# blyssprivacy/sdk

Hardware: NVIDIA H100
Metric: PIR server queries/sec (Spiral process_query) (higher is better)
Workload: dtype u64

## Files before the change

### sdk_b200/build.py

```python
import os
import subprocess
import sys

HERE = os.path.dirname(os.path.abspath(__file__))
CSRC = os.path.join(HERE, "csrc")
SO = os.path.join(HERE, "libb200pir.so")
SOURCES = ["api.cu", "poly_kernels.cu", "mul_kernels.cu", "imma_kernels.cu", "wire_kernels.cu", "tc5_kernels.cu", "dpir_gemm.cu"]
HEADERS = ["common.cuh", "kernels.h", "ntt_core.cuh", "tc5_layout.cuh", "tc5_ptx.cuh", "ntt_core4096.cuh", "ntt_tables.hpp", os.path.join("..", "..", "include", "b200pir.h")]
NVCC_FLAGS = ["-gencode", "arch=compute_90a,code=sm_90a", "-lineinfo", "-O3", "-std=c++17", "--extended-lambda",
              "-Xcompiler", "-fPIC", "-ccbin", "/usr/bin/g++" if os.path.exists("/usr/bin/g++") else "g++"]


def _stale():
    if not os.path.exists(SO):
        return True
    t = os.path.getmtime(SO)
    return any(os.path.getmtime(os.path.join(CSRC, f)) > t for f in SOURCES + HEADERS)


def build(force=False, verbose=False):
    if not force and not _stale():
        return SO
    nvcc = os.environ.get("NVCC", "/usr/local/cuda/bin/nvcc")
    objs = []
    procs = []
    for src in SOURCES:
        obj = os.path.join(CSRC, src.replace(".cu", ".o"))
        cmd = [nvcc] + NVCC_FLAGS + (["-Xptxas", "-v"] if verbose else []) + ["-c", os.path.join(CSRC, src), "-o", obj]
        procs.append((src, subprocess.Popen(cmd, stdout=subprocess.PIPE, stderr=subprocess.STDOUT, text=True)))
        objs.append(obj)
    for src, p in procs:
        out, _ = p.communicate()
        if verbose or p.returncode:
            sys.stderr.write(out)
        if p.returncode:
            raise RuntimeError("nvcc failed on " + src)
    subprocess.check_call([nvcc, "-shared", "-gencode", "arch=compute_90a,code=sm_90a", "-o", SO] + objs + ["-ccbin", NVCC_FLAGS[-1]])
    return SO


if __name__ == "__main__":
# ... 2 lines not shown
```

### sdk_b200/csrc/poly_kernels.cu

```cuda
#include "kernels.h"
#include "ntt_core4096.cuh"

namespace b200pir {

namespace {

constexpr int CTA = 512;
constexpr int HI_TW = NTT_N - 64;

__constant__ Twiddle c_tw_lo[2][3][64];

struct TwConst {
  int n, dir;
  __device__ __forceinline__ Twiddle operator()(int i) const { return c_tw_lo[n][dir][i]; }
  __device__ __forceinline__ void load2(int i, Twiddle (&t)[2]) const { t[0] = (*this)(i); t[1] = (*this)(i + 1); }
  __device__ __forceinline__ void load4(int i, Twiddle (&t)[4]) const {
    t[0] = (*this)(i); t[1] = (*this)(i + 1); t[2] = (*this)(i + 2); t[3] = (*this)(i + 3);
  }
};
struct TwShared {
  const Twiddle* p;
  __device__ __forceinline__ Twiddle operator()(int i) const { return p[i - 64]; }
  __device__ __forceinline__ void load2(int i, Twiddle (&t)[2]) const {
    uint4 v = *reinterpret_cast<const uint4*>(p + (i - 64));
    t[0] = Twiddle{v.x, v.y}; t[1] = Twiddle{v.z, v.w};
  }
  __device__ __forceinline__ void load4(int i, Twiddle (&t)[4]) const {
    uint4 v = *reinterpret_cast<const uint4*>(p + (i - 64)), w = *(reinterpret_cast<const uint4*>(p + (i - 64)) + 1);
    t[0] = Twiddle{v.x, v.y}; t[1] = Twiddle{v.z, v.w}; t[2] = Twiddle{w.x, w.y}; t[3] = Twiddle{w.z, w.w};
  }
};
struct TwGlobal {
  const Twiddle* p;
  __device__ __forceinline__ Twiddle operator()(int i) const {
// ... 140 lines not shown
#pragma unroll
        for (int e = 0; e < 8; e++) acc[r][e] += (uint64_t)x1[e] * cv[e];
      }
    }
  }
#pragma unroll 1
  for (; k < ndig; k++) {
    uint32_t x[8];
#pragma unroll
    for (int a = 0; a < 8; a++) x[a] = gadget_digit_fast<BYTE>(v(a), k, bits, mask);
    if (SM) ntt_forward_group_lz<NTT_OUT_LAZY16>(g.tid, x, g.smem, TwConst{g.n, 0}, TwShared{g.fwd_hi_sm}, g.q, CtaSync());
    else ntt_forward_group_lz<NTT_OUT_LAZY16>(g.tid, x, g.smem, TwConst{g.n, 0}, TwGlobal{g.fwd}, g.q, CtaSync());
    if (cnt + 1 > 16) { acc_reduce<ROWS>(acc, g); cnt = 1; }
    cnt += 1;
    const uint32_t* c = c0 + (size_t)k * col_step;
#pragma unroll
    for (int r = 0; r < ROWS; r++) {
      uint32_t cv[8];
      ld8_ro(cv, c + (size_t)r * row_step);
#pragma unroll
      for (int e = 0; e < 8; e++) acc[r][e] += (uint64_t)x[e] * cv[e];
    }
  }
}

template <int ROWS, bool SM, typename Coef>
__device__ __forceinline__ void digits_mac(uint64_t (&acc)[ROWS][8], int& cnt, Coef v, int ndig,
                                           int bits, const uint32_t* c0, size_t col_step, size_t row_step,
                                           const Grp& g) {
  if (bits == 8) digits_mac_impl<ROWS, SM, true>(acc, cnt, v, ndig, bits, c0, col_step, row_step, g);
  else digits_mac_impl<ROWS, SM, false>(acc, cnt, v, ndig, bits, c0, col_step, row_step, g);
}

template <typename Sink>
__device__ __forceinline__ void crt_lift(const uint32_t (&x)[8], uint32_t* res, const Grp& g, const DevParams& P,
                                         Sink sink) {
  __syncthreads();
#pragma unroll
  for (int a = 0; a < 8; a++) res[g.n * POLY + a * 256 + g.tid] = x[a];
  __syncthreads();
#pragma unroll
  for (int a4 = 0; a4 < 4; a4++) {
    int z = (g.n * 4 + a4) * 256 + g.tid;
    sink(z, crt_compose(res[z], res[POLY + z], P));
  }
}

__global__ void __launch_bounds__(256) k_ntt32(DevParams P, uint32_t* polys, int inverse) {
  __shared__ __align__(16) uint32_t ntt_smem[NTT_SMEM_WORDS];
  Grp g = make_grp_single(P, ntt_smem, blockIdx.y);
  uint32_t* p = polys + ((size_t)blockIdx.x * 2 + g.n) * POLY;
  uint32_t x[8];
  if (!inverse) {
#pragma unroll
    for (int a = 0; a < 8; a++) x[a] = p[a * 256 + g.tid];
    grp_ntt_fwd<false>(g, x);
    st8(p + g.tid * 8, x);
  } else {
    ld8(x, p + g.tid * 8);
    grp_ntt_inv(g, x);
#pragma unroll
    for (int a = 0; a < 8; a++) p[a * 256 + g.tid] = x[a];
  }
}
__global__ void __launch_bounds__(NTT4K_THREADS)
k_ntt32_4k(uint32_t q0, uint32_t q1, const Twiddle* __restrict__ tw , uint32_t* polys, int inverse) {
// ... 106 lines not shown
    const uint64_t* ct = base + (size_t)(src == 0 ? i : half + i) * 2 * POLY;
    const uint32_t* C = (src == 0 ? c_neg : c_pos) + qoff;
#pragma unroll 1
    for (int rho = 0; rho < 2; rho++) {
      uint64_t v[8];
#pragma unroll
      for (int a = 0; a < 8; a++) v[a] = ct[rho * POLY + a * 256 + g.tid];
      const uint32_t* c0 = C + ((size_t)rho * 2 + g.n) * POLY + g.tid * 8;
      digits_mac<2, false>(acc, cnt, RegCoef{v}, t_gsw, bits, c0, col_step, row_step, g);
    }
  }
  uint64_t* dst = base + (size_t)i * 2 * POLY;
#pragma unroll 1
  for (int r = 0; r < 2; r++) {
    uint32_t x[8];
#pragma unroll
    for (int e = 0; e < 8; e++) x[e] = barrett64(acc[r][e], g.cr1, g.q);
    grp_ntt_inv(g, x);
    uint64_t* d = dst + r * POLY;
    crt_lift(x, res, g, P, [&](int z, uint64_t val) { d[z] = val; });
  }
}

__device__ __forceinline__ uint32_t digit_diff(uint64_t vh, uint64_t vi, int k, int bits, uint64_t mask, uint32_t q) {
  return gadget_digit(vh, k, bits, mask) - gadget_digit(vi, k, bits, mask) + q;
}
__device__ __forceinline__ uint32_t byte_pair_diff(uint64_t vh, uint64_t vi, int k) {
  const uint32_t sel = 0x7070u | ((uint32_t)(k + 1) << 8) | (uint32_t)k;
  return __byte_perm((uint32_t)vh, (uint32_t)(vh >> 32), sel) + 0x01000100u -
         __byte_perm((uint32_t)vi, (uint32_t)(vi >> 32), sel);
}
constexpr int kFoldPlanes = 4;

template <bool BYTE>
__global__ void __launch_bounds__(256, 2)
k_fold_res_lz(DevParams P, const uint32_t* __restrict__ in, uint32_t* __restrict__ out, size_t batch_stride, int half,
              const uint32_t* __restrict__ c_pos, size_t c_batch_stride, int slices_per_query, int t_gsw, int bits,
              const uint32_t* __restrict__ zero_flags ) {
  if (zero_flags) {
    const int bz = blockIdx.x / half, iz = blockIdx.x % half;
    const uint32_t fa = zero_flags[(size_t)bz * 2 * half + iz], fb = zero_flags[(size_t)bz * 2 * half + half + iz];
    if (fa | fb) {
      const uint32_t* src = in + (size_t)bz * batch_stride + (size_t)((fa ? half : 0) + iz) * 4 * POLY;
      uint32_t* dst = out + (size_t)bz * batch_stride + (size_t)iz * 4 * POLY;
#pragma unroll
      for (int rho = 0; rho < 2; rho++) {
        uint32_t x[8];
        ld8_ro(x, src + ((size_t)rho * 2 + blockIdx.y) * POLY + threadIdx.x * 8);
        st8(dst + ((size_t)rho * 2 + blockIdx.y) * POLY + threadIdx.x * 8, x);
      }
      return;
    }
  }
  extern __shared__ __align__(16) uint8_t dyn_smem[];
  uint32_t* sm0 = reinterpret_cast<uint32_t*>(dyn_smem);
  uint32_t* sm1 = sm0 + NTT_SMEM_WORDS;
  Twiddle* tw = reinterpret_cast<Twiddle*>(sm1 + NTT_SMEM_WORDS);
  Grp g = make_grp_single(P, sm0, blockIdx.y);
  stage_fwd_twiddles(g, tw);
  const TwConst lo{g.n, 0};
  const TwShared hi{tw};
  const int b = blockIdx.x / half, i = blockIdx.x % half;
  const uint32_t* ci = in + (size_t)b * batch_stride + (size_t)i * 4 * POLY;
  const uint32_t* ch = in + (size_t)b * batch_stride + (size_t)(half + i) * 4 * POLY;
  const uint32_t* C = c_pos + (size_t)(b / slices_per_query) * c_batch_stride;
  const int cols = 2 * t_gsw;
  const size_t row_step = (size_t)cols * 2 * POLY;
  const uint64_t mask = (1ull << bits) - 1;
  const uint32_t q = g.q;
  uint32_t* planes = reinterpret_cast<uint32_t*>(tw + HI_TW) + g.tid;

  uint64_t acc[2][8];
#pragma unroll
  for (int r = 0; r < 2; r++)
#pragma unroll
    for (int e = 0; e < 8; e++) acc[r][e] = 0;
  int cnt = 0;
#pragma unroll 1
  for (int rho = 0; rho < 2; rho++) {
    uint64_t vi[8], vh[8];
#pragma unroll
    for (int a = 0; a < 8; a++) {
      const int z = a * 256 + g.tid;
      vi[a] = crt_compose(__ldg(ci + (rho * 2 + 0) * POLY + z), __ldg(ci + (rho * 2 + 1) * POLY + z), P);
      vh[a] = crt_compose(__ldg(ch + (rho * 2 + 0) * POLY + z), __ldg(ch + (rho * 2 + 1) * POLY + z), P);
      if (BYTE) {
#pragma unroll
        for (int p = 0; p < kFoldPlanes; p++)
          if (2 * p < t_gsw) planes[p * POLY + a * 256] = byte_pair_diff(vh[a], vi[a], 2 * p);
      }
    }
    const uint32_t* c0 = C + ((size_t)rho * 2 + g.n) * POLY + g.tid * 8;
    int k = 0;
#pragma unroll 1
    for (; k + 1 < t_gsw; k += 2) {
      uint32_t x0[8], x1[8];
#pragma unroll
      for (int a = 0; a < 8; a++) {
        if (BYTE) {
          const uint32_t w = planes[(k >> 1) * POLY + a * 256];
          x0[a] = (w & 0xffffu) + (q - 256u);
          x1[a] = (w >> 16) + (q - 256u);
        } else {
          x0[a] = digit_diff(vh[a], vi[a], k, bits, mask, q);
          x1[a] = digit_diff(vh[a], vi[a], k + 1, bits, mask, q);
        }
      }
      ntt_forward_group2_lz<NTT_OUT_LAZY16>(g.tid, x0, x1, sm0, sm1, lo, hi, q, CtaSync());
      if (cnt + 2 > 16) { acc_reduce<2>(acc, g); cnt = 1; }
      cnt += 2;
#pragma unroll
      for (int r = 0; r < 2; r++) {
        uint32_t cv[8];
        ld8_ro(cv, c0 + (size_t)r * row_step + (size_t)k * 4 * POLY);
#pragma unroll
        for (int e = 0; e < 8; e++) acc[r][e] += (uint64_t)x0[e] * cv[e];
      }
#pragma unroll
      for (int r = 0; r < 2; r++) {
        uint32_t cv[8];
        ld8_ro(cv, c0 + (size_t)r * row_step + (size_t)(k + 1) * 4 * POLY);
#pragma unroll
        for (int e = 0; e < 8; e++) acc[r][e] += (uint64_t)x1[e] * cv[e];
      }
    }
    if (k < t_gsw) {
      uint32_t x0[8];
#pragma unroll
      for (int a = 0; a < 8; a++)
        x0[a] = BYTE ? (planes[(k >> 1) * POLY + a * 256] & 0xffffu) + (q - 256u) : digit_diff(vh[a], vi[a], k, bits, mask, q);
      ntt_forward_group_lz<NTT_OUT_LAZY16>(g.tid, x0, sm0, lo, hi, q, CtaSync());
      if (cnt + 1 > 16) { acc_reduce<2>(acc, g); cnt = 1; }
      cnt += 1;
#pragma unroll
      for (int r = 0; r < 2; r++) {
        uint32_t cv[8];
        ld8_ro(cv, c0 + (size_t)r * row_step + (size_t)k * 4 * POLY);
#pragma unroll
        for (int e = 0; e < 8; e++) acc[r][e] += (uint64_t)x0[e] * cv[e];
      }
    }
  }
  uint32_t y0[8], y1[8];
#pragma unroll
  for (int e = 0; e < 8; e++) {
    y0[e] = barrett64(acc[0][e], g.cr1, q);
    y1[e] = barrett64(acc[1][e], g.cr1, q);
  }
  ntt_inverse_group2_nh(g.tid, y0, y1, sm0, sm1, TwConst{g.n, 2}, TwGlobal{g.inv_lz}, q, CtaSync());
  uint32_t* co = out + (size_t)b * batch_stride + (size_t)i * 4 * POLY;
#pragma unroll
  for (int a = 0; a < 8; a++) {
    const int z = a * 256 + g.tid;
    co[(0 * 2 + g.n) * POLY + z] = addmod(y0[a], __ldg(ci + (0 * 2 + g.n) * POLY + z), q);
    co[(1 * 2 + g.n) * POLY + z] = addmod(y1[a], __ldg(ci + (1 * 2 + g.n) * POLY + z), q);
  }
}

__global__ void __launch_bounds__(256)
k_ct_zero_flags(const uint32_t* __restrict__ cts, size_t batch_stride, int per_batch, uint32_t* __restrict__ flags) {
  const int b = blockIdx.x / per_batch, idx = blockIdx.x % per_batch;
  const uint4* p = reinterpret_cast<const uint4*>(cts + (size_t)b * batch_stride + (size_t)idx * 4 * POLY);
  uint32_t acc = 0;
#pragma unroll
  for (int k = 0; k < 8; k++) {
    const uint4 v = __ldg(p + k * 256 + threadIdx.x);
    acc |= v.x | v.y | v.z | v.w;
  }
  const int any = __syncthreads_or(acc != 0);
  if (threadIdx.x == 0) flags[blockIdx.x] = any ? 0u : 1u;
}

__global__ void k_folding_neg(DevParams P, uint32_t* out, const uint32_t* vf, size_t total, int t_gsw, int bits) {
  size_t idx = (size_t)blockIdx.x * blockDim.x + threadIdx.x;
  if (idx >= total) return;
  int n = (int)((idx / POLY) & 1);
  size_t poly = idx / (2 * POLY);
  int cols = 2 * t_gsw;
  int c = (int)(poly % cols);
  int r = (int)((poly / cols) & 1);
  uint32_t q = P.q[n];
  uint32_t v = vf[idx];
  uint32_t neg = v == 0 ? 0u : q - v;
  uint32_t gval = 0;
  if ((c & 1) == r) {
    int j = c >> 1;
    if (bits * j < 64) gval = barrett64(1ull << (bits * j), P.cr1[n], q);
  }
  out[idx] = addmod(neg, gval, q);
// ... 186 lines not shown
            const unsigned ee = 2u * (__brev(sidx) >> (32 - NTT_LOG_N)) + 1u;
            const unsigned e2 = (ee * (unsigned)R.t_auto) & (2u * POLY - 1u);
            const unsigned src = __brev((e2 - 1u) >> 1) >> (32 - NTT_LOG_N);
            yy = barrett64((uint64_t)yy * __ldg(ng + src), g.cr1, g.q);
          }
          s = addmod(s, yy, g.q);
        }
        o[e] = s;
      }
      st8(dst + ((size_t)rho * 2 + g.n) * POLY + g.tid * 8, o);
    }
    __syncthreads();
  }
}

__global__ void __launch_bounds__(256)
k_expand_intt(DevParams P, const uint32_t* __restrict__ v, size_t v_stride, uint32_t* __restrict__ xr, size_t xr_stride,
              ExpandRound R) {
  __shared__ __align__(16) uint32_t ntt_smem[NTT_SMEM_WORDS];
  const int i = blockIdx.x;
  if ((R.stop_round > 0 && R.r > R.stop_round && (i & 1)) ||
      (R.stop_round > 0 && R.r == R.stop_round && (i & 1) && (i / 2) >= R.max_bits_to_gen_right))
    return;
  Grp g = make_grp_single(P, ntt_smem, blockIdx.y);
  const uint32_t* src = v + (size_t)blockIdx.z * v_stride + ((size_t)i * 4 + g.n) * POLY;
  uint32_t x[8];
  ld8_ro(x, src + g.tid * 8);
  grp_ntt_inv(g, x);
  uint32_t* dst = xr + (size_t)blockIdx.z * xr_stride + ((size_t)i * 2 + g.n) * POLY;
#pragma unroll
  for (int a = 0; a < 8; a++) dst[a * 256 + g.tid] = x[a];
}

__global__ void __launch_bounds__(256, 2)
k_expand_round_res(DevParams P, uint32_t* v, size_t v_stride, const uint32_t* __restrict__ xr, size_t xr_stride,
                   ExpandRound R, const uint32_t* __restrict__ neg1) {
  v += (size_t)blockIdx.z * v_stride;
  xr += (size_t)blockIdx.z * xr_stride;
  extern __shared__ __align__(16) uint8_t dyn_smem[];
  uint32_t* sm0 = reinterpret_cast<uint32_t*>(dyn_smem);
  uint32_t* sm1 = sm0 + NTT_SMEM_WORDS;
  uint64_t* autom = reinterpret_cast<uint64_t*>(sm1 + NTT_SMEM_WORDS);
  Twiddle* tw = reinterpret_cast<Twiddle*>(autom + POLY);
  Grp g = make_grp_single(P, sm0, blockIdx.y);
  g.smem2 = sm1;
  const int i = blockIdx.x;
  const uint32_t* ng = neg1 + (size_t)g.n * POLY;
  uint32_t* vi = v + (size_t)i * 4 * POLY;
  uint32_t* vo = v + (size_t)(i + R.num_in) * 4 * POLY;
  if ((R.stop_round > 0 && R.r > R.stop_round && (i & 1)) ||
      (R.stop_round > 0 && R.r == R.stop_round && (i & 1) && (i / 2) >= R.max_bits_to_gen_right)) {
    if (R.fill_skipped) {
      uint32_t nn[8];
      ld8_ro(nn, ng + g.tid * 8);
#pragma unroll
      for (int rho = 0; rho < 2; rho++) {
        uint32_t x[8];
        ld8(x, vi + ((size_t)rho * 2 + g.n) * POLY + g.tid * 8);
#pragma unroll
        for (int e = 0; e < 8; e++) x[e] = barrett64((uint64_t)x[e] * nn[e], g.cr1, g.q);
        st8(vo + ((size_t)rho * 2 + g.n) * POLY + g.tid * 8, x);
      }
    }
    return;
  }
  const bool left = (R.r != 0) && ((i & 1) == 0);
  const uint32_t* W = left ? R.tab_left[blockIdx.z] + R.off_left : R.tab_right[blockIdx.z] + R.off_right;
  const int t_exp = left ? R.t_left : R.t_right;
  const int bits = left ? R.bits_left : R.bits_right;
  stage_fwd_twiddles(g, tw);
  const uint32_t* x0r = xr + (size_t)i * 2 * POLY;
  const uint32_t* x1r = x0r + POLY;
  const uint32_t* row1 = vi + ((size_t)2 + g.n) * POLY;
  const uint64_t Q = P.modulus;
  const uint32_t q0 = P.q[0], q1 = P.q[1];
#pragma unroll 1
  for (int half = 1; half >= 0; half--) {
    const int shift = half ? R.num_in : 0;
#pragma unroll
    for (int a = 0; a < 8; a++) {
      const int k = a * 256 + g.tid;
      const int zs = (k + shift) & (POLY - 1);
      uint32_t a0 = __ldg(x0r + zs), a1 = __ldg(x1r + zs);
      if (k + shift >= POLY) {
        a0 = a0 ? q0 - a0 : 0u;
        a1 = a1 ? q1 - a1 : 0u;
      }
      const uint64_t val = crt_compose(a0, a1, P);
      const unsigned prod = (unsigned)k * (unsigned)R.t_auto;
      const unsigned num = prod >> NTT_LOG_N, rem = prod & (POLY - 1);
      autom[rem] = (num & 1u) ? Q - val : val;
    }
    __syncthreads();
    uint64_t acc[2][8];
#pragma unroll
    for (int r = 0; r < 2; r++)
#pragma unroll
      for (int e = 0; e < 8; e++) acc[r][e] = 0;
    int cnt = 0;
    digits_mac<2, true>(acc, cnt, SmemCoef{autom + g.tid}, t_exp, bits, W + (size_t)g.n * POLY + g.tid * 8, (size_t)2 * POLY,
                        (size_t)t_exp * 2 * POLY, g);
    uint32_t yy[8];
#pragma unroll
    for (int e = 0; e < 8; e++) {
      const unsigned sidx = (unsigned)(g.tid * 8 + e);
      const unsigned ee = 2u * (__brev(sidx) >> (32 - NTT_LOG_N)) + 1u;
      const unsigned e2 = (ee * (unsigned)R.t_auto) & (2u * POLY - 1u);
      const unsigned src = __brev((e2 - 1u) >> 1) >> (32 - NTT_LOG_N);
      uint32_t t = row1[src];
      if (half) t = barrett64((uint64_t)t * __ldg(ng + src), g.cr1, g.q);
      yy[e] = t;
    }
    __syncthreads();
    uint32_t* dst = half ? vo : vi;
    uint32_t nn[8];
    if (half) ld8_ro(nn, ng + g.tid * 8);
#pragma unroll
    for (int rho = 0; rho < 2; rho++) {
      uint32_t o[8];
      ld8(o, vi + ((size_t)rho * 2 + g.n) * POLY + g.tid * 8);
#pragma unroll
      for (int e = 0; e < 8; e++) {
        uint32_t base = o[e];
        if (half) base = barrett64((uint64_t)base * nn[e], g.cr1, g.q);
        uint32_t s = addmod(base, barrett64(acc[rho][e], g.cr1, g.q), g.q);
        o[e] = rho ? addmod(s, yy[e], g.q) : s;
      }
      st8(dst + ((size_t)rho * 2 + g.n) * POLY + g.tid * 8, o);
    }
  }
}

__global__ void k_reorient(MulGeom G, uint4* q_dev, size_t q_stride, const uint32_t* v, size_t v_stride, int idx_factor) {
  q_dev += (size_t)blockIdx.y * q_stride;
  v += (size_t)blockIdx.y * v_stride;
  size_t idx = (size_t)blockIdx.x * blockDim.x + threadIdx.x;
  if (idx >= (size_t)G.dim0 * POLY) return;
  int z = (int)(idx % POLY), j = (int)(idx / POLY);
  const uint32_t* ct = v + (size_t)idx_factor * j * 4 * POLY;
  uint4 o = make_uint4(ct[z], ct[POLY + z], ct[2 * POLY + z], ct[3 * POLY + z]);
  q_dev[((size_t)(j >> 1) * 2 + (j & 1)) * POLY + z] = o;
}

__global__ void __launch_bounds__(CTA, 1)
k_regev_to_gsw(DevParams P, uint32_t* v_gsw, size_t gsw_stride, const uint32_t* v, size_t v_stride, int idx_factor,
               int idx_offset, const uint32_t* const* tab_conv, int t_gsw, int t_conv, int bits_conv) {
  const uint32_t* v_conv = tab_conv[blockIdx.y];
  v_gsw += (size_t)blockIdx.y * gsw_stride;
  v += (size_t)blockIdx.y * v_stride;
  extern __shared__ __align__(16) uint8_t dyn_smem[];
  uint32_t* ntt_smem = reinterpret_cast<uint32_t*>(dyn_smem);
  uint32_t* res = ntt_smem + 4 * NTT_SMEM_WORDS;
  uint64_t* raw = reinterpret_cast<uint64_t*>(res + 2 * POLY);
  Twiddle* tw = reinterpret_cast<Twiddle*>(raw + 2 * POLY);
  Grp g = make_grp(P, ntt_smem);
  g.smem2 = ntt_smem + (2 + g.n) * NTT_SMEM_WORDS;
  stage_fwd_twiddles(g, tw + g.n * HI_TW);
  const int i = blockIdx.x / t_gsw, j = blockIdx.x % t_gsw;
  const int idx_inp = idx_factor * (i * t_gsw + j) + idx_offset;
  const uint32_t* inp = v + (size_t)idx_inp * 4 * POLY;
  const int cols = 2 * t_gsw;
  uint32_t* out = v_gsw + (size_t)i * 2 * cols * 2 * POLY;
#pragma unroll 1
// ... 157 lines not shown
  const uint64_t inst_bits = first_cnt * q2_bits + rest_cnt * q1_bits;
  uint64_t lo_bit = (uint64_t)w * 64, hi_bit = lo_bit + 64;
  uint64_t word = 0;
  uint64_t bit = lo_bit;
  while (bit < hi_bit) {
    uint64_t inst = bit / inst_bits;
    if (inst >= (uint64_t)instances) break;
    uint64_t off = bit - inst * inst_bits;
    const uint64_t* pk = packed + inst * (uint64_t)(n + 1) * n * POLY;
    uint64_t vstart, val;
    int vb;
    if (off < first_cnt * q2_bits) {
      uint64_t vi = off / q2_bits;
      vstart = inst * inst_bits + vi * q2_bits;
      vb = q2_bits;
      val = rescale_dev(pk[vi], P.modulus, q2);
    } else {
      uint64_t o2 = off - first_cnt * q2_bits;
      uint64_t vi = o2 / q1_bits;
      vstart = inst * inst_bits + first_cnt * q2_bits + vi * q1_bits;
      vb = q1_bits;
      val = rescale_dev(pk[first_cnt + vi], P.modulus, q1);
    }
    val &= (vb >= 64) ? ~0ull : ((1ull << vb) - 1);
    if (vstart >= lo_bit) word |= val << (vstart - lo_bit);
    else word |= val >> (lo_bit - vstart);
    bit = vstart + vb;
  }
  out[w] = word;
}

inline unsigned grid1d(size_t total, int block) { return (unsigned)((total + block - 1) / block); }
const size_t kDynSmemBig = (size_t)(4 * NTT_SMEM_WORDS + 2 * POLY) * 4 + (size_t)2 * POLY * 8 + (size_t)2 * HI_TW * 8;
const size_t kDynSmemFold = (size_t)(2 * NTT_SMEM_WORDS) * 4 + (size_t)HI_TW * 8;

}

void upload_poly_constants(const Twiddle* lo ) {
  B200_CUDA(cudaMemcpyToSymbol(c_tw_lo, lo, sizeof(Twiddle) * 2 * 3 * 64));
}
void launch_ntt_u64(const DevParams& P, uint64_t* polys, size_t count, bool inverse, cudaStream_t s) {
  if (count) ++g_kernel_launches, k_ntt_u64<<<dim3((unsigned)count, 2), 256, 0, s>>>(P, polys, inverse ? 1 : 0);
}
void launch_ntt32(const DevParams& P, uint32_t* polys, size_t count, bool inverse, cudaStream_t s) {
  if (count) ++g_kernel_launches, k_ntt32<<<dim3((unsigned)count, 2), 256, 0, s>>>(P, polys, inverse ? 1 : 0);
}
void launch_ntt32_4k(uint32_t q0, uint32_t q1, const Twiddle* tw, uint32_t* polys, size_t count, bool inverse, cudaStream_t s) {
  if (count) ++g_kernel_launches, k_ntt32_4k<<<dim3((unsigned)count, 2), NTT4K_THREADS, 0, s>>>(q0, q1, tw, polys, inverse ? 1 : 0);
}
void launch_to_ntt(const DevParams& P, uint32_t* out, const uint64_t* raw, size_t count, cudaStream_t s) {
  if (count) ++g_kernel_launches, k_to_ntt<<<dim3((unsigned)count, 2), 256, 0, s>>>(P, out, raw, 0, 0);
}
void launch_to_ntt_strided(const DevParams& P, uint32_t* out, size_t out_stride, const uint64_t* raw, size_t raw_stride,
                           size_t count, int batches, cudaStream_t s) {
  if (count && batches)
    ++g_kernel_launches, k_to_ntt<<<dim3((unsigned)count, 2, (unsigned)batches), 256, 0, s>>>(P, out, raw, out_stride, raw_stride);
}
void launch_raw_to_res(const DevParams& P, uint32_t* out, const uint64_t* raw, size_t polys, cudaStream_t s) {
  if (polys) ++g_kernel_launches, k_raw_to_res<<<grid1d(polys * POLY, 256), 256, 0, s>>>(P, out, raw, polys);
}
void launch_res_to_raw(const DevParams& P, uint64_t* out, const uint32_t* res, size_t polys, cudaStream_t s) {
  if (polys) ++g_kernel_launches, k_res_to_raw<<<grid1d(polys * POLY, 256), 256, 0, s>>>(P, out, res, polys);
}
void launch_fold_res(const DevParams& P, const uint32_t* in, uint32_t* out, size_t batch, size_t batch_stride, int half,
                     const uint32_t* c_pos, size_t c_batch_stride, int slices_per_query, int t_gsw, int bits,
                     uint32_t* zero_flags, cudaStream_t s) {
  if (batch == 0 || half == 0) return;
  if (zero_flags) {
    ++g_kernel_launches;
    k_ct_zero_flags<<<(unsigned)(batch * 2 * half), 256, 0, s>>>(in, batch_stride, 2 * half, zero_flags);
  }
  ++g_kernel_launches;
  const dim3 grid((unsigned)(batch * half), 2);
  const bool byte = bits == 8 && t_gsw <= 2 * kFoldPlanes;
  const size_t smem = kDynSmemFold + (byte ? (size_t)kFoldPlanes * POLY * 4 : 0);
  auto kern = byte ? k_fold_res_lz<true> : k_fold_res_lz<false>;
  opt_in_smem(kern, (int)smem);
  kern<<<grid, 256, smem, s>>>(P, in, out, batch_stride, half, c_pos, c_batch_stride, slices_per_query, t_gsw, bits, zero_flags);
}
void launch_from_ntt(const DevParams& P, uint64_t* out_raw, const uint32_t* in, size_t count, cudaStream_t s) {
  if (count) ++g_kernel_launches, k_from_ntt<<<(unsigned)count, CTA, 0, s>>>(P, out_raw, in);
}
void launch_widen(uint64_t* out, const uint32_t* in, size_t words, cudaStream_t s) {
  if (words) ++g_kernel_launches, k_widen<<<grid1d(words, 256), 256, 0, s>>>(out, in, words);
}
void launch_narrow(uint32_t* out, const uint64_t* in, size_t words, cudaStream_t s) {
  if (words) ++g_kernel_launches, k_narrow<<<grid1d(words, 256), 256, 0, s>>>(out, in, words);
}
void launch_fold_round(const DevParams& P, uint64_t* cts, size_t batch, size_t batch_stride, int half,
                       const uint32_t* c_pos, const uint32_t* c_neg, size_t c_batch_stride, int slices_per_query,
                       int t_gsw, int bits, cudaStream_t s) {
  if (batch == 0 || half == 0) return;
  ++g_kernel_launches;
  k_fold_round<<<(unsigned)(batch * half), CTA, 0, s>>>(P, cts, batch_stride, half, c_pos, c_neg, c_batch_stride,
                                                        slices_per_query, t_gsw, bits);
}
void launch_folding_neg(const DevParams& P, uint32_t* out, const uint32_t* v_folding, int count, int t_gsw, int bits,
                        cudaStream_t s) {
  size_t total = (size_t)count * 2 * 2 * t_gsw * 2 * POLY;
  if (total) ++g_kernel_launches, k_folding_neg<<<grid1d(total, 256), 256, 0, s>>>(P, out, v_folding, total, t_gsw, bits);
}
void launch_expand_scalar(const DevParams& P, uint32_t* v, size_t v_stride, int nq, int num_in, const uint32_t* neg1_r,
                          cudaStream_t s) {
  size_t total = (size_t)num_in * 4 * POLY;
  ++g_kernel_launches;
  k_expand_scalar<<<dim3(grid1d(total, 256), nq), 256, 0, s>>>(P, v, v_stride, num_in, neg1_r);
}
void launch_expand_round(const DevParams& P, uint32_t* v, size_t v_stride, int nq, const ExpandRound& R, cudaStream_t s) {
  opt_in_smem(k_expand_round, (int)kDynSmemBig);
  ++g_kernel_launches;
  k_expand_round<<<dim3((unsigned)(2 * R.num_in), nq), CTA, kDynSmemBig, s>>>(P, v, v_stride, R);
}
void launch_expand_round_pair(const DevParams& P, uint32_t* v, size_t v_stride, int nq, const ExpandRound& R,
                              const uint32_t* neg1_r, cudaStream_t s) {
  opt_in_smem(k_expand_round_pair, (int)kDynSmemBig);
  ++g_kernel_launches;
  k_expand_round_pair<<<dim3((unsigned)R.num_in, nq), CTA, kDynSmemBig, s>>>(P, v, v_stride, R, neg1_r);
}
void launch_expand_round_res(const DevParams& P, uint32_t* v, size_t v_stride, uint32_t* xr, size_t xr_stride, int nq,
                             const ExpandRound& R, const uint32_t* neg1_r, cudaStream_t s) {
  const size_t smem = (size_t)2 * NTT_SMEM_WORDS * 4 + (size_t)POLY * 8 + (size_t)HI_TW * 8;
  opt_in_smem(k_expand_round_res, (int)smem);
  g_kernel_launches += 2;
  k_expand_intt<<<dim3((unsigned)R.num_in, 2, nq), 256, 0, s>>>(P, v, v_stride, xr, xr_stride, R);
  k_expand_round_res<<<dim3((unsigned)R.num_in, 2, nq), 256, smem, s>>>(P, v, v_stride, xr, xr_stride, R, neg1_r);
}
void launch_reorient(const MulGeom& G, uint4* q_dev, size_t q_stride, const uint32_t* v, size_t v_stride, int nq,
                     int idx_factor, cudaStream_t s) {
  size_t total = (size_t)G.dim0 * POLY;
  ++g_kernel_launches;
  k_reorient<<<dim3(grid1d(total, 256), nq), 256, 0, s>>>(G, q_dev, q_stride, v, v_stride, idx_factor);
}
void launch_regev_to_gsw(const DevParams& P, uint32_t* v_gsw, size_t gsw_stride, const uint32_t* v, size_t v_stride,
                         int nq, int count, int idx_factor, int idx_offset, const uint32_t* const* tab_conv, int t_gsw,
                         int t_conv, int bits_conv, cudaStream_t s) {
  if (count == 0) return;
  opt_in_smem(k_regev_to_gsw, (int)kDynSmemBig);
  ++g_kernel_launches;
  k_regev_to_gsw<<<dim3((unsigned)(count * t_gsw), nq), CTA, kDynSmemBig, s>>>(P, v_gsw, gsw_stride, v, v_stride,
                                                                               idx_factor, idx_offset, tab_conv, t_gsw,
                                                                               t_conv, bits_conv);
}
template <int ROWS>
static void launch_pack_t(const DevParams& P, uint64_t* out_raw, size_t out_q_stride, const uint32_t* folded,
                          size_t ct_stride, size_t in_q_stride, int nq, const uint32_t* const* tab_pack, int instances,
                          int t_conv, int bits_conv, int version, cudaStream_t s) {
  opt_in_smem(k_pack<ROWS>, (int)kDynSmemBig);
  ++g_kernel_launches;
  k_pack<ROWS><<<dim3((unsigned)(instances * (ROWS - 1)), nq), CTA, kDynSmemBig, s>>>(
      P, out_raw, out_q_stride, folded, ct_stride, in_q_stride, tab_pack, t_conv, bits_conv, version);
}
void launch_pack(const DevParams& P, uint64_t* out_raw, size_t out_q_stride, const uint32_t* folded, size_t ct_stride,
                 size_t in_q_stride, int nq, const uint32_t* const* tab_pack, int n, int instances, int t_conv, int bits_conv,
                 int version, cudaStream_t s) {
// ... 18 lines not shown
```

Baseline: 1234.

## Use warp-level NTTs for gadget digits in fold and expand kernels

```diff
diff --git a/sdk_b200/build.py b/sdk_b200/build.py
--- a/sdk_b200/build.py
+++ b/sdk_b200/build.py
@@ -6,7 +6,7 @@
 CSRC = os.path.join(HERE, "csrc")
 SO = os.path.join(HERE, "libb200pir.so")
 SOURCES = ["api.cu", "poly_kernels.cu", "mul_kernels.cu", "imma_kernels.cu", "wire_kernels.cu", "tc5_kernels.cu", "dpir_gemm.cu"]
-HEADERS = ["common.cuh", "kernels.h", "ntt_core.cuh", "tc5_layout.cuh", "tc5_ptx.cuh", "ntt_core4096.cuh", "ntt_tables.hpp", os.path.join("..", "..", "include", "b200pir.h")]
+HEADERS = ["common.cuh", "kernels.h", "ntt_core.cuh", "tc5_layout.cuh", "tc5_ptx.cuh", "ntt_core4096.cuh", "ntt_warp.cuh", "ntt_tables.hpp", os.path.join("..", "..", "include", "b200pir.h")]
 NVCC_FLAGS = ["-gencode", "arch=compute_90a,code=sm_90a", "-lineinfo", "-O3", "-std=c++17", "--extended-lambda",
               "-Xcompiler", "-fPIC", "-ccbin", "/usr/bin/g++" if os.path.exists("/usr/bin/g++") else "g++"]
 
diff --git a/sdk_b200/csrc/ntt_warp.cuh b/sdk_b200/csrc/ntt_warp.cuh
--- /dev/null
+++ b/sdk_b200/csrc/ntt_warp.cuh
@@ -0,0 +1,121 @@
+#pragma once
+#include "ntt_core.cuh"
+
+namespace b200pir {
+
+static const uint32_t kNttModuli[2] = {268369921u, 249561089u};
+template <int N> struct NttMod { static constexpr uint32_t q = N ? 249561089u : 268369921u; };
+
+static const int NTTW_WORDS = NTT_N;
+static const int NTTW_TW_PAIRS = 992;
+
+NTT_HD int nttw_phys(int e) { return e ^ ((e >> 6) & 31); }
+NTT_HD int nttw_chunk(int c) { return c ^ (((c >> 4) & 7) ^ ((c >> 3) & 1)); }
+
+NTT_HD int nttw_pair_index(int s, int p, int lane) { return 32 * ((1 << s) - 1) + 32 * p + lane; }
+NTT_HD int nttw_pair_entry(int u) {
+  int s = 0;
+  while (u >= 32 * ((2 << s) - 1)) s++;
+  const int r = u - 32 * ((1 << s) - 1), p = r >> 5, lane = r & 31;
+  return (64 << s) + (2 << s) * lane + 2 * p;
+}
+
+#if defined(__CUDA_ARCH__)
+NTT_HD void nttw_ld_pair(const Twiddle* tw2, int u, Twiddle& a, Twiddle& b) {
+  const uint4 v = *reinterpret_cast<const uint4*>(tw2 + 2 * u);
+  a = Twiddle{v.x, v.y};
+  b = Twiddle{v.z, v.w};
+}
+NTT_HD void nttw_st_chunk(uint32_t* buf, int c, uint32_t v0, uint32_t v1, uint32_t v2, uint32_t v3) {
+  *reinterpret_cast<uint4*>(buf + 4 * nttw_chunk(c)) = make_uint4(v0, v1, v2, v3);
+}
+#else
+NTT_HD void nttw_ld_pair(const Twiddle* tw2, int u, Twiddle& a, Twiddle& b) { a = tw2[2 * u]; b = tw2[2 * u + 1]; }
+NTT_HD void nttw_st_chunk(uint32_t* buf, int c, uint32_t v0, uint32_t v1, uint32_t v2, uint32_t v3) {
+  uint32_t* p = buf + 4 * nttw_chunk(c);
+  p[0] = v0; p[1] = v1; p[2] = v2; p[3] = v3;
+}
+#endif
+
+template <int MM, typename TabLo>
+NTT_HD void nttw_phase1_stage(uint32_t (&x)[64], TabLo lo, uint32_t q) {
+  constexpr int t = 32 >> MM;
+#pragma unroll
+  for (int i = 0; i < (1 << MM); i++) {
+    const Twiddle w = lo((1 << MM) + i);
+#pragma unroll
+    for (int j = 0; j < t; j++) bfly_fwd_lz(x[2 * i * t + j], x[2 * i * t + j + t], w, q, 2 * q);
+  }
+}
+template <typename TabLo>
+NTT_HD void nttw_fwd_phase1(int lane, uint32_t (&x)[64], uint32_t* buf, TabLo lo, uint32_t q) {
+  nttw_phase1_stage<0>(x, lo, q);
+  nttw_phase1_stage<1>(x, lo, q);
+  nttw_phase1_stage<2>(x, lo, q);
+  nttw_phase1_stage<3>(x, lo, q);
+  nttw_phase1_stage<4>(x, lo, q);
+  nttw_phase1_stage<5>(x, lo, q);
+#pragma unroll
+  for (int a = 0; a < 64; a++) buf[nttw_phys(32 * a + lane)] = x[a];
+}
+
+template <int S>
+NTT_HD void nttw_phase2_stage(int lane, int h, uint32_t (&y)[32], const Twiddle* tw2, uint32_t q) {
+  constexpr int d = 16 >> S;
+#pragma unroll
+  for (int p = 0; p < (1 << (S - 1)); p++) {
+    Twiddle w[2];
+    nttw_ld_pair(tw2, nttw_pair_index(S, (h << (S - 1)) + p, lane), w[0], w[1]);
+#pragma unroll
+    for (int g2 = 0; g2 < 2; g2++) {
+      const int g = 2 * p + g2;
+#pragma unroll
+      for (int j = 0; j < d; j++) bfly_fwd_lz(y[2 * g * d + j], y[2 * g * d + j + d], w[g2], q, 2 * q);
+    }
+  }
+}
+NTT_HD void nttw_fwd_phase2_half(int lane, int h, uint32_t* buf, const Twiddle* tw2, uint32_t q) {
+  const uint32_t two_q = 2 * q;
+  uint32_t y[32];
+#pragma unroll
+  for (int b = 0; b < 32; b++) y[b] = buf[64 * lane + ((32 * h + b) ^ lane)];
+  {
+    Twiddle w[2];
+    nttw_ld_pair(tw2, nttw_pair_index(0, 0, lane), w[0], w[1]);
+#pragma unroll
+    for (int b = 0; b < 16; b++) bfly_fwd_lz(y[b], y[b + 16], w[h], q, two_q);
+#pragma unroll
+    for (int b = 0; b < 32; b++) y[b] = ntt_c8(y[b], 8 * q);
+  }
+  nttw_phase2_stage<1>(lane, h, y, tw2, q);
+  nttw_phase2_stage<2>(lane, h, y, tw2, q);
+  nttw_phase2_stage<3>(lane, h, y, tw2, q);
+  nttw_phase2_stage<4>(lane, h, y, tw2, q);
+#pragma unroll
+  for (int c = 0; c < 8; c++) nttw_st_chunk(buf, 16 * lane + 8 * h + c, y[4 * c], y[4 * c + 1], y[4 * c + 2], y[4 * c + 3]);
+}
+
+#if defined(__CUDACC__)
+__device__ __forceinline__ void nttw_stage_twiddles(const Twiddle* fwd, Twiddle* dst) {
+  for (int u = threadIdx.x; u < NTTW_TW_PAIRS; u += blockDim.x) {
+    const uint4 v = __ldg(reinterpret_cast<const uint4*>(fwd + nttw_pair_entry(u)));
+    *reinterpret_cast<uint4*>(dst + 2 * u) = v;
+  }
+}
+
+template <int N, typename TabLo>
+__device__ __forceinline__ void nttw_forward(int lane, uint32_t (&x)[64], uint32_t* buf, TabLo lo, const Twiddle* tw2) {
+  constexpr uint32_t q = NttMod<N>::q;
+  nttw_fwd_phase1(lane, x, buf, lo, q);
+  __syncwarp();
+  nttw_fwd_phase2_half(lane, 0, buf, tw2, q);
+  nttw_fwd_phase2_half(lane, 1, buf, tw2, q);
+}
+__device__ __forceinline__ void nttw_load8(uint32_t (&y)[8], const uint32_t* buf, int t) {
+  const uint4 a = *reinterpret_cast<const uint4*>(buf + 4 * nttw_chunk(2 * t));
+  const uint4 b = *reinterpret_cast<const uint4*>(buf + 4 * nttw_chunk(2 * t + 1));
+  y[0] = a.x; y[1] = a.y; y[2] = a.z; y[3] = a.w; y[4] = b.x; y[5] = b.y; y[6] = b.z; y[7] = b.w;
+}
+#endif
+
+}
diff --git a/sdk_b200/csrc/poly_kernels.cu b/sdk_b200/csrc/poly_kernels.cu
--- a/sdk_b200/csrc/poly_kernels.cu
+++ b/sdk_b200/csrc/poly_kernels.cu
@@ -1,5 +1,6 @@
 #include "kernels.h"
 #include "ntt_core4096.cuh"
+#include "ntt_warp.cuh"
 
 namespace b200pir {
 
@@ -206,6 +207,49 @@
   else digits_mac_impl<ROWS, SM, false>(acc, cnt, v, ndig, bits, c0, col_step, row_step, g);
 }
 
+constexpr int kDigitWarps = 8;
+constexpr size_t kWarpBufBytes = (size_t)kDigitWarps * NTTW_WORDS * 4;
+constexpr size_t kTw2Bytes = (size_t)NTTW_TW_PAIRS * 16;
+template <int N, typename Digit>
+__device__ __forceinline__ void warp_digits_mac(uint64_t (&acc)[2][8], int& cnt, int ndig, Digit digit, uint32_t* bufs,
+                                                const Twiddle* tw2, const uint32_t* c0, int col_step, int row_step,
+                                                uint64_t cr1) {
+  constexpr uint32_t q = NttMod<N>::q;
+  const int tid = threadIdx.x, warp = tid >> 5, lane = tid & 31;
+#pragma unroll 1
+  for (int k0 = 0; k0 < ndig; k0 += kDigitWarps) {
+    __syncthreads();
+    if (k0 + warp < ndig) {
+      uint32_t x[64];
+      digit(k0 + warp, lane, x);
+      nttw_forward<N>(lane, x, bufs + warp * NTTW_WORDS, TwConst{N, 0}, tw2);
+    }
+    __syncthreads();
+    const int nd = min(kDigitWarps, ndig - k0);
+    if (cnt + nd > 16) {
+#pragma unroll
+      for (int r = 0; r < 2; r++)
+#pragma unroll
+        for (int e = 0; e < 8; e++) acc[r][e] = barrett64(acc[r][e], cr1, q);
+      cnt = 1;
+    }
+    cnt += nd;
+#pragma unroll 2
+    for (int j = 0; j < nd; j++) {
+      uint32_t y[8];
+      nttw_load8(y, bufs + j * NTTW_WORDS, tid);
+      const uint32_t* c = c0 + (k0 + j) * col_step;
+#pragma unroll
+      for (int r = 0; r < 2; r++) {
+        uint32_t cv[8];
+        ld8_ro(cv, c + r * row_step);
+#pragma unroll
+        for (int e = 0; e < 8; e++) acc[r][e] += (uint64_t)y[e] * cv[e];
+      }
+    }
+  }
+}
+
 template <typename Sink>
 __device__ __forceinline__ void crt_lift(const uint32_t (&x)[8], uint32_t* res, const Grp& g, const DevParams& P,
                                          Sink sink) {
@@ -378,13 +422,86 @@
 }
 constexpr int kFoldPlanes = 4;
 
+template <bool BYTE, int N>
+__device__ __forceinline__ void fold_res_lz(const DevParams& P, const uint32_t* __restrict__ in, uint32_t* __restrict__ out,
+                                            size_t batch_stride, int half, const uint32_t* __restrict__ c_pos,
+                                            size_t c_batch_stride, int slices_per_query, int t_gsw, int bits,
+                                            uint8_t* dyn_smem) {
+  constexpr uint32_t q = NttMod<N>::q;
+  uint32_t* bufs = reinterpret_cast<uint32_t*>(dyn_smem);
+  uint32_t* sm0 = bufs;
+  uint32_t* sm1 = bufs + NTT_SMEM_WORDS;
+  Twiddle* tw2 = reinterpret_cast<Twiddle*>(bufs + kDigitWarps * NTTW_WORDS);
+  uint32_t* src = reinterpret_cast<uint32_t*>(tw2 + 2 * NTTW_TW_PAIRS);
+  uint64_t* src64 = reinterpret_cast<uint64_t*>(src);
+  nttw_stage_twiddles(P.fwd[N], tw2);
+  const int tid = threadIdx.x;
+  const uint64_t cr1 = P.cr1[N];
+  const int step = blockIdx.x >> 1, b = step / half, i = step % half;
+  const uint32_t* ci = in + (size_t)b * batch_stride + (size_t)i * 4 * POLY;
+  const int row_step = 2 * t_gsw * 2 * POLY;
+
+  uint64_t acc[2][8];
+#pragma unroll
+  for (int r = 0; r < 2; r++)
+#pragma unroll
+    for (int e = 0; e < 8; e++) acc[r][e] = 0;
+  int cnt = 0;
+#pragma unroll 1
+  for (int rho = 0; rho < 2; rho++) {
+    const uint32_t* ch = ci + (size_t)half * 4 * POLY;
+#pragma unroll
+    for (int a = 0; a < 8; a++) {
+      const int z = a * 256 + tid;
+      const uint64_t vi = crt_compose(__ldg(ci + (rho * 2 + 0) * POLY + z), __ldg(ci + (rho * 2 + 1) * POLY + z), P);
+      const uint64_t vh = crt_compose(__ldg(ch + (rho * 2 + 0) * POLY + z), __ldg(ch + (rho * 2 + 1) * POLY + z), P);
+      if (BYTE) {
+#pragma unroll
+        for (int p = 0; p < kFoldPlanes; p++)
+          if (2 * p < t_gsw) src[p * POLY + z] = byte_pair_diff(vh, vi, 2 * p);
+      } else {
+        src64[z] = vi;
+        src64[POLY + z] = vh;
+      }
+    }
+    auto digit = [&](int k, int lane, uint32_t (&x)[64]) {
+      if (BYTE) {
+        const uint32_t* pl = src + (k >> 1) * POLY + lane;
+        const int sh = (k & 1) * 16;
+#pragma unroll
+        for (int a = 0; a < 64; a++) x[a] = ((pl[32 * a] >> sh) & 0xffffu) + (q - 256u);
+      } else {
+        const uint64_t mask = (1ull << bits) - 1;
+#pragma unroll
+        for (int a = 0; a < 64; a++) x[a] = digit_diff(src64[POLY + 32 * a + lane], src64[32 * a + lane], k, bits, mask, q);
+      }
+    };
+    const uint32_t* C = c_pos + (size_t)(b / slices_per_query) * c_batch_stride + ((size_t)rho * 2 + N) * POLY;
+    warp_digits_mac<N>(acc, cnt, t_gsw, digit, bufs, tw2, C + tid * 8, 4 * POLY, row_step, cr1);
+  }
+  uint32_t y0[8], y1[8];
+#pragma unroll
+  for (int e = 0; e < 8; e++) {
+    y0[e] = barrett64(acc[0][e], cr1, q);
+    y1[e] = barrett64(acc[1][e], cr1, q);
+  }
+  ntt_inverse_group2_nh(tid, y0, y1, sm0, sm1, TwConst{N, 2}, TwGlobal{P.inv_lz[N]}, q, CtaSync());
+  uint32_t* co = out + (size_t)b * batch_stride + (size_t)i * 4 * POLY;
+#pragma unroll
+  for (int a = 0; a < 8; a++) {
+    const int z = a * 256 + tid;
+    co[(0 * 2 + N) * POLY + z] = addmod(y0[a], __ldg(ci + (0 * 2 + N) * POLY + z), q);
+    co[(1 * 2 + N) * POLY + z] = addmod(y1[a], __ldg(ci + (1 * 2 + N) * POLY + z), q);
+  }
+}
 template <bool BYTE>
 __global__ void __launch_bounds__(256, 2)
 k_fold_res_lz(DevParams P, const uint32_t* __restrict__ in, uint32_t* __restrict__ out, size_t batch_stride, int half,
               const uint32_t* __restrict__ c_pos, size_t c_batch_stride, int slices_per_query, int t_gsw, int bits,
               const uint32_t* __restrict__ zero_flags ) {
+  const int n = blockIdx.x & 1, step = blockIdx.x >> 1;
   if (zero_flags) {
-    const int bz = blockIdx.x / half, iz = blockIdx.x % half;
+    const int bz = step / half, iz = step % half;
     const uint32_t fa = zero_flags[(size_t)bz * 2 * half + iz], fb = zero_flags[(size_t)bz * 2 * half + half + iz];
     if (fa | fb) {
       const uint32_t* src = in + (size_t)bz * batch_stride + (size_t)((fa ? half : 0) + iz) * 4 * POLY;
@@ -392,115 +509,17 @@
 #pragma unroll
       for (int rho = 0; rho < 2; rho++) {
         uint32_t x[8];
-        ld8_ro(x, src + ((size_t)rho * 2 + blockIdx.y) * POLY + threadIdx.x * 8);
-        st8(dst + ((size_t)rho * 2 + blockIdx.y) * POLY + threadIdx.x * 8, x);
+        ld8_ro(x, src + ((size_t)rho * 2 + n) * POLY + threadIdx.x * 8);
+        st8(dst + ((size_t)rho * 2 + n) * POLY + threadIdx.x * 8, x);
       }
       return;
     }
   }
   extern __shared__ __align__(16) uint8_t dyn_smem[];
-  uint32_t* sm0 = reinterpret_cast<uint32_t*>(dyn_smem);
-  uint32_t* sm1 = sm0 + NTT_SMEM_WORDS;
-  Twiddle* tw = reinterpret_cast<Twiddle*>(sm1 + NTT_SMEM_WORDS);
-  Grp g = make_grp_single(P, sm0, blockIdx.y);
-  stage_fwd_twiddles(g, tw);
-  const TwConst lo{g.n, 0};
-  const TwShared hi{tw};
-  const int b = blockIdx.x / half, i = blockIdx.x % half;
-  const uint32_t* ci = in + (size_t)b * batch_stride + (size_t)i * 4 * POLY;
-  const uint32_t* ch = in + (size_t)b * batch_stride + (size_t)(half + i) * 4 * POLY;
-  const uint32_t* C = c_pos + (size_t)(b / slices_per_query) * c_batch_stride;
-  const int cols = 2 * t_gsw;
-  const size_t row_step = (size_t)cols * 2 * POLY;
-  const uint64_t mask = (1ull << bits) - 1;
-  const uint32_t q = g.q;
-  uint32_t* planes = reinterpret_cast<uint32_t*>(tw + HI_TW) + g.tid;
-
-  uint64_t acc[2][8];
-#pragma unroll
-  for (int r = 0; r < 2; r++)
-#pragma unroll
-    for (int e = 0; e < 8; e++) acc[r][e] = 0;
-  int cnt = 0;
-#pragma unroll 1
-  for (int rho = 0; rho < 2; rho++) {
-    uint64_t vi[8], vh[8];
-#pragma unroll
-    for (int a = 0; a < 8; a++) {
-      const int z = a * 256 + g.tid;
-      vi[a] = crt_compose(__ldg(ci + (rho * 2 + 0) * POLY + z), __ldg(ci + (rho * 2 + 1) * POLY + z), P);
-      vh[a] = crt_compose(__ldg(ch + (rho * 2 + 0) * POLY + z), __ldg(ch + (rho * 2 + 1) * POLY + z), P);
-      if (BYTE) {
-#pragma unroll
-        for (int p = 0; p < kFoldPlanes; p++)
-          if (2 * p < t_gsw) planes[p * POLY + a * 256] = byte_pair_diff(vh[a], vi[a], 2 * p);
-      }
-    }
-    const uint32_t* c0 = C + ((size_t)rho * 2 + g.n) * POLY + g.tid * 8;
-    int k = 0;
-#pragma unroll 1
-    for (; k + 1 < t_gsw; k += 2) {
-      uint32_t x0[8], x1[8];
-#pragma unroll
-      for (int a = 0; a < 8; a++) {
-        if (BYTE) {
-          const uint32_t w = planes[(k >> 1) * POLY + a * 256];
-          x0[a] = (w & 0xffffu) + (q - 256u);
-          x1[a] = (w >> 16) + (q - 256u);
-        } else {
-          x0[a] = digit_diff(vh[a], vi[a], k, bits, mask, q);
-          x1[a] = digit_diff(vh[a], vi[a], k + 1, bits, mask, q);
-        }
-      }
-      ntt_forward_group2_lz<NTT_OUT_LAZY16>(g.tid, x0, x1, sm0, sm1, lo, hi, q, CtaSync());
-      if (cnt + 2 > 16) { acc_reduce<2>(acc, g); cnt = 1; }
-      cnt += 2;
-#pragma unroll
-      for (int r = 0; r < 2; r++) {
-        uint32_t cv[8];
-        ld8_ro(cv, c0 + (size_t)r * row_step + (size_t)k * 4 * POLY);
-#pragma unroll
-        for (int e = 0; e < 8; e++) acc[r][e] += (uint64_t)x0[e] * cv[e];
-      }
-#pragma unroll
-      for (int r = 0; r < 2; r++) {
-        uint32_t cv[8];
-        ld8_ro(cv, c0 + (size_t)r * row_step + (size_t)(k + 1) * 4 * POLY);
-#pragma unroll
-        for (int e = 0; e < 8; e++) acc[r][e] += (uint64_t)x1[e] * cv[e];
-      }
-    }
-    if (k < t_gsw) {
-      uint32_t x0[8];
-#pragma unroll
-      for (int a = 0; a < 8; a++)
-        x0[a] = BYTE ? (planes[(k >> 1) * POLY + a * 256] & 0xffffu) + (q - 256u) : digit_diff(vh[a], vi[a], k, bits, mask, q);
-      ntt_forward_group_lz<NTT_OUT_LAZY16>(g.tid, x0, sm0, lo, hi, q, CtaSync());
-      if (cnt + 1 > 16) { acc_reduce<2>(acc, g); cnt = 1; }
-      cnt += 1;
-#pragma unroll
-      for (int r = 0; r < 2; r++) {
-        uint32_t cv[8];
-        ld8_ro(cv, c0 + (size_t)r * row_step + (size_t)k * 4 * POLY);
-#pragma unroll
-        for (int e = 0; e < 8; e++) acc[r][e] += (uint64_t)x0[e] * cv[e];
-      }
-    }
-  }
-  uint32_t y0[8], y1[8];
-#pragma unroll
-  for (int e = 0; e < 8; e++) {
-    y0[e] = barrett64(acc[0][e], g.cr1, q);
-    y1[e] = barrett64(acc[1][e], g.cr1, q);
-  }
-  ntt_inverse_group2_nh(g.tid, y0, y1, sm0, sm1, TwConst{g.n, 2}, TwGlobal{g.inv_lz}, q, CtaSync());
-  uint32_t* co = out + (size_t)b * batch_stride + (size_t)i * 4 * POLY;
-#pragma unroll
-  for (int a = 0; a < 8; a++) {
-    const int z = a * 256 + g.tid;
-    co[(0 * 2 + g.n) * POLY + z] = addmod(y0[a], __ldg(ci + (0 * 2 + g.n) * POLY + z), q);
-    co[(1 * 2 + g.n) * POLY + z] = addmod(y1[a], __ldg(ci + (1 * 2 + g.n) * POLY + z), q);
-  }
+  if (n == 0)
+    fold_res_lz<BYTE, 0>(P, in, out, batch_stride, half, c_pos, c_batch_stride, slices_per_query, t_gsw, bits, dyn_smem);
+  else
+    fold_res_lz<BYTE, 1>(P, in, out, batch_stride, half, c_pos, c_batch_stride, slices_per_query, t_gsw, bits, dyn_smem);
 }
 
 __global__ void __launch_bounds__(256)
@@ -753,18 +772,13 @@
   for (int a = 0; a < 8; a++) dst[a * 256 + g.tid] = x[a];
 }
 
-__global__ void __launch_bounds__(256, 2)
-k_expand_round_res(DevParams P, uint32_t* v, size_t v_stride, const uint32_t* __restrict__ xr, size_t xr_stride,
-                   ExpandRound R, const uint32_t* __restrict__ neg1) {
-  v += (size_t)blockIdx.z * v_stride;
-  xr += (size_t)blockIdx.z * xr_stride;
-  extern __shared__ __align__(16) uint8_t dyn_smem[];
-  uint32_t* sm0 = reinterpret_cast<uint32_t*>(dyn_smem);
-  uint32_t* sm1 = sm0 + NTT_SMEM_WORDS;
-  uint64_t* autom = reinterpret_cast<uint64_t*>(sm1 + NTT_SMEM_WORDS);
-  Twiddle* tw = reinterpret_cast<Twiddle*>(autom + POLY);
-  Grp g = make_grp_single(P, sm0, blockIdx.y);
-  g.smem2 = sm1;
+template <int N>
+__device__ __forceinline__ void expand_round_res(const DevParams& P, uint32_t* v, const uint32_t* __restrict__ xr,
+                                                 const ExpandRound& R, const uint32_t* __restrict__ neg1, uint8_t* dyn_smem) {
+  uint32_t* bufs = reinterpret_cast<uint32_t*>(dyn_smem);
+  uint64_t* autom = reinterpret_cast<uint64_t*>(bufs + kDigitWarps * NTTW_WORDS);
+  Twiddle* tw2 = reinterpret_cast<Twiddle*>(autom + POLY);
+  Grp g = make_grp_single(P, bufs, N);
   const int i = blockIdx.x;
   const uint32_t* ng = neg1 + (size_t)g.n * POLY;
   uint32_t* vi = v + (size_t)i * 4 * POLY;
@@ -789,7 +803,8 @@
   const uint32_t* W = left ? R.tab_left[blockIdx.z] + R.off_left : R.tab_right[blockIdx.z] + R.off_right;
   const int t_exp = left ? R.t_left : R.t_right;
   const int bits = left ? R.bits_left : R.bits_right;
-  stage_fwd_twiddles(g, tw);
+  const uint64_t mask = (1ull << bits) - 1;
+  nttw_stage_twiddles(P.fwd[N], tw2);
   const uint32_t* x0r = xr + (size_t)i * 2 * POLY;
   const uint32_t* x1r = x0r + POLY;
   const uint32_t* row1 = vi + ((size_t)2 + g.n) * POLY;
@@ -812,15 +827,24 @@
       const unsigned num = prod >> NTT_LOG_N, rem = prod & (POLY - 1);
       autom[rem] = (num & 1u) ? Q - val : val;
     }
-    __syncthreads();
     uint64_t acc[2][8];
 #pragma unroll
     for (int r = 0; r < 2; r++)
 #pragma unroll
       for (int e = 0; e < 8; e++) acc[r][e] = 0;
     int cnt = 0;
-    digits_mac<2, true>(acc, cnt, SmemCoef{autom + g.tid}, t_exp, bits, W + (size_t)g.n * POLY + g.tid * 8, (size_t)2 * POLY,
-                        (size_t)t_exp * 2 * POLY, g);
+    auto digit = [&](int k, int lane, uint32_t (&x)[64]) {
+      const uint64_t* c = autom + lane;
+      if (bits == 8) {
+#pragma unroll
+        for (int a = 0; a < 64; a++) x[a] = gadget_digit_fast<true>(c[32 * a], k, bits, mask);
+      } else {
+#pragma unroll
+        for (int a = 0; a < 64; a++) x[a] = gadget_digit_fast<false>(c[32 * a], k, bits, mask);
+      }
+    };
+    warp_digits_mac<N>(acc, cnt, t_exp, digit, bufs, tw2, W + (size_t)N * POLY + g.tid * 8, 2 * POLY,
+                       t_exp * 2 * POLY, g.cr1);
     uint32_t yy[8];
 #pragma unroll
     for (int e = 0; e < 8; e++) {
@@ -850,6 +874,16 @@
       st8(dst + ((size_t)rho * 2 + g.n) * POLY + g.tid * 8, o);
     }
   }
+}
+
+__global__ void __launch_bounds__(256, 2)
+k_expand_round_res(DevParams P, uint32_t* v, size_t v_stride, const uint32_t* __restrict__ xr, size_t xr_stride,
+                   ExpandRound R, const uint32_t* __restrict__ neg1) {
+  extern __shared__ __align__(16) uint8_t dyn_smem[];
+  v += (size_t)blockIdx.z * v_stride;
+  xr += (size_t)blockIdx.z * xr_stride;
+  if (blockIdx.y == 0) expand_round_res<0>(P, v, xr, R, neg1, dyn_smem);
+  else expand_round_res<1>(P, v, xr, R, neg1, dyn_smem);
 }
 
 __global__ void k_reorient(MulGeom G, uint4* q_dev, size_t q_stride, const uint32_t* v, size_t v_stride, int idx_factor) {
@@ -1073,7 +1107,6 @@
 
 inline unsigned grid1d(size_t total, int block) { return (unsigned)((total + block - 1) / block); }
 const size_t kDynSmemBig = (size_t)(4 * NTT_SMEM_WORDS + 2 * POLY) * 4 + (size_t)2 * POLY * 8 + (size_t)2 * HI_TW * 8;
-const size_t kDynSmemFold = (size_t)(2 * NTT_SMEM_WORDS) * 4 + (size_t)HI_TW * 8;
 
 }
 
@@ -1112,9 +1145,9 @@
     k_ct_zero_flags<<<(unsigned)(batch * 2 * half), 256, 0, s>>>(in, batch_stride, 2 * half, zero_flags);
   }
   ++g_kernel_launches;
-  const dim3 grid((unsigned)(batch * half), 2);
+  const dim3 grid((unsigned)(batch * half * 2));
   const bool byte = bits == 8 && t_gsw <= 2 * kFoldPlanes;
-  const size_t smem = kDynSmemFold + (byte ? (size_t)kFoldPlanes * POLY * 4 : 0);
+  const size_t smem = kWarpBufBytes + kTw2Bytes + (size_t)kFoldPlanes * POLY * 4;
   auto kern = byte ? k_fold_res_lz<true> : k_fold_res_lz<false>;
   opt_in_smem(kern, (int)smem);
   kern<<<grid, 256, smem, s>>>(P, in, out, batch_stride, half, c_pos, c_batch_stride, slices_per_query, t_gsw, bits, zero_flags);
@@ -1160,7 +1193,7 @@
 }
 void launch_expand_round_res(const DevParams& P, uint32_t* v, size_t v_stride, uint32_t* xr, size_t xr_stride, int nq,
                              const ExpandRound& R, const uint32_t* neg1_r, cudaStream_t s) {
-  const size_t smem = (size_t)2 * NTT_SMEM_WORDS * 4 + (size_t)POLY * 8 + (size_t)HI_TW * 8;
+  const size_t smem = kWarpBufBytes + (size_t)POLY * 8 + kTw2Bytes;
   opt_in_smem(k_expand_round_res, (int)smem);
   g_kernel_launches += 2;
   k_expand_intt<<<dim3((unsigned)R.num_in, 2, nq), 256, 0, s>>>(P, v, v_stride, xr, xr_stride, R);
```

Result: faster. 1256, median of 6 (+1.8%).
